# HenryHZY/VL-PET

Measured on AMD Instinct MI355X. Metric: multitask samples/sec (BART-base, r=96), higher is better.
Workload: dtype bf16

## Files before the change

### include/vlpet_hip.h

```cpp
#ifndef VLPET_HIP_H
#define VLPET_HIP_H
#include <stddef.h>
#include <stdint.h>

#ifdef __cplusplus
extern "C" {
#endif

#define VLPET_F32 0
#define VLPET_BF16 1

#define VLPET_E_SHAPE (-1)
#define VLPET_E_RANK (-2)
#define VLPET_E_ALIGN (-3)
#define VLPET_E_WORKSPACE (-4)
#define VLPET_E_NULL (-5)
#define VLPET_E_DTYPE (-6)
#define VLPET_E_ALIAS (-7)

#define VLPET_GATE_NONE 0
#define VLPET_GATE_MUL 1
#define VLPET_GATE_ADD 2

typedef void* vlpet_stream_t;
// ... 302 lines not shown
                      int64_t bs_v, const void* k_new, const void* v_new, int64_t ld_new, int pos, const uint8_t* key_mask,
                      int64_t ld_mask, const float* bias, int64_t ld_bias, void* o, int64_t ld_o, int B, int H, int D, int Lk,
                      float scale, int io_dtype, vlpet_stream_t stream);
int vlpet_greedy_pick(const void* logits, int64_t ld, int V, int64_t* ids, int64_t ld_ids, int pos, int* unfinished, int* counter,
                      int B, int eos_token_id, int pad_token_id, int min_length, int no_repeat_ngram_size, int io_dtype,
                      vlpet_stream_t stream);

int vlpet_attn_decode_beam(const void* q, int64_t ld_q, void* k_cache, void* v_cache, int64_t ld_k, int64_t bs_k, int64_t ld_v,
                           int64_t bs_v, const void* k_new, const void* v_new, int64_t ld_new, int pos, const uint8_t* key_mask,
                           int64_t ld_mask, const float* bias, int64_t ld_bias, void* o, int64_t ld_o, int B, int H, int D,
                           int Lk, float scale, int group, const int* key_rows, int64_t ld_key_rows, int io_dtype,
                           vlpet_stream_t stream);
int vlpet_beam_rows(const void* logits, int64_t ld, int V, const int64_t* ids, int64_t ld_ids, int pos, int rows, int num_beams,
                    int slices, int eos_token_id, int min_length, int no_repeat_ngram_size, int force_eos, float* part_stats,
                    float* part_val, int* part_tok, int io_dtype, vlpet_stream_t stream);
int vlpet_beam_advance(const float* part_stats, const float* part_val, const int* part_tok, int slices, int V, int B, int num_beams,
                       float* beam_scores, const int64_t* ids_in, int64_t* ids_out, int64_t ld_ids, const int* key_rows_in,
                       int* key_rows_out, int64_t ld_key_rows, int64_t* next_tokens, float* hyp_score, int* hyp_meta,
                       int64_t* hyp_tokens, int64_t ld_hyp, float* item_worst, int* item_state, int* counter, int pos,
                       int eos_token_id, int pad_token_id, float length_penalty, int early_stopping, vlpet_stream_t stream);

int vlpet_attn_decode_at(const void* q, int64_t ld_q, void* k_cache, void* v_cache, int64_t ld_k, int64_t bs_k, int64_t ld_v,
                         int64_t bs_v, const void* k_new, const void* v_new, int64_t ld_new, const int* pos_dev, int pos_limit,
                         const uint8_t* key_mask, int64_t ld_mask, const float* bias, int64_t ld_bias, int64_t pos_stride_bias,
                         void* o, int64_t ld_o, int B, int H, int D, int Lk, float scale, const int* key_rows,
                         int64_t ld_key_rows, int64_t parity_stride_key_rows, int io_dtype, vlpet_stream_t stream);
int vlpet_greedy_pick_at(const void* logits, int64_t ld, int V, int64_t* ids, int64_t ld_ids, const int* pos_dev, int pos_limit,
                         int* unfinished, int* counters, int64_t* next_tokens, int B, int eos_token_id, int pad_token_id,
                         int min_length, int no_repeat_ngram_size, int io_dtype, vlpet_stream_t stream);
int vlpet_beam_rows_at(const void* logits, int64_t ld, int V, const int64_t* ids, int64_t ld_ids, int64_t parity_stride_ids,
                       const int* pos_dev, int pos_limit, int rows, int num_beams, int slices, int eos_token_id, int min_length,
                       int no_repeat_ngram_size, int force_eos_pos, float* part_stats, float* part_val, int* part_tok,
                       int io_dtype, vlpet_stream_t stream);
int vlpet_beam_advance_at(const float* part_stats, const float* part_val, const int* part_tok, int slices, int V, int B,
                          int num_beams, float* beam_scores, int64_t* ids, int64_t ld_ids, int64_t parity_stride_ids,
                          int* key_rows, int64_t ld_key_rows, int64_t parity_stride_key_rows, int64_t* next_tokens,
                          float* hyp_score, int* hyp_meta, int64_t* hyp_tokens, int64_t ld_hyp, float* item_worst, int* item_state,
                          int* counters, const int* pos_dev, int pos_limit, int eos_token_id, int pad_token_id,
                          float length_penalty, int early_stopping, vlpet_stream_t stream);

int vlpet_adapter_tail_rows(void);
int vlpet_adapter_tail_applies(int64_t M, int d, int r, int io_dtype);
int vlpet_adapter_tail_fwd(const void* h, const void* res, const void* down_w, const void* down_b, const void* up_w,
                           const void* up_b, const float* gamma, const float* beta, void* out, int64_t M, int d, int r,
                           float scale, float eps, int norm_mode, int param_dtype, int io_dtype, vlpet_stream_t stream);

size_t vlpet_phm_workspace_bytes(int d, int r, int n);
int vlpet_phm_expand_pair_fwd(const void* rule_d, const void* W_d, const void* rule_u, const void* W_u, void* wt_d, void* wt_u,
                              int d, int r, int n, int param_dtype, vlpet_stream_t stream);
int vlpet_phm_expand_pair_bwd(const float* dwt_d, const float* dwt_u, const void* rule_d, const void* W_d, const void* rule_u,
                              const void* W_u, float* drule_d, float* dW_d, float* drule_u, float* dW_u, void* workspace,
                              size_t workspace_bytes, int d, int r, int n, int param_dtype, vlpet_stream_t stream);

#ifdef __cplusplus
}
#endif
#endif
```

### vl-pet_amd/_lib.py

```python
from __future__ import annotations

import ctypes
import os
from ctypes import c_char_p, c_float, c_int, c_int64, c_size_t, c_uint64, c_void_p

_HERE = os.path.dirname(os.path.abspath(__file__))
LIB_PATH = os.environ.get("VLPET_LIB") or os.path.join(_HERE, "lib", "libvlpet_hip.so")

VLPET_F32 = 0
VLPET_BF16 = 1
GATE_NONE, GATE_MUL, GATE_ADD = 0, 1, 2

_lib = None

SIGNATURES = {
    "vlpet_version": (c_int, []),
    "vlpet_error_string": (c_char_p, [c_int]),
    "vlpet_rank_tiles": (c_int, [c_int]),
    "vlpet_packed_bytes": (c_size_t, [c_int, c_int, c_int]),
    "vlpet_pack_pair": (c_int, [c_void_p, c_void_p, c_int, c_void_p, c_void_p, c_int, c_int, c_int, c_int, c_int,
                                c_void_p, c_void_p]),
    "vlpet_pack_pairs": (c_int, [c_int, c_void_p, c_void_p, c_int, c_void_p, c_void_p, c_int, c_int, c_int, c_int, c_int,
                                 c_void_p, c_void_p]),
    "vlpet_adapter_gate_fwd": (c_int, [c_void_p, c_void_p, c_void_p, c_void_p, c_void_p, c_int64, c_int, c_int,
# ... 99 lines not shown
    "vlpet_attn_bwd": (c_int, [c_void_p] * 10 + [c_int] * 5 + [c_float, c_float, c_uint64, c_void_p]),
    "vlpet_attn_fwd_ld": (c_int, [c_void_p] * 7 + [c_int] * 7 + [c_float, c_float, c_uint64, c_void_p]),
    "vlpet_attn_bwd_ld": (c_int, [c_void_p] * 10 + [c_int] * 7 + [c_float, c_float, c_uint64, c_void_p]),
    "vlpet_attn_fwd_bias": (c_int, [c_void_p] * 8 + [c_int] * 7 + [c_float, c_float, c_uint64, c_void_p]),
    "vlpet_attn_bwd_bias": (c_int, [c_void_p] * 12 + [c_int] * 7 + [c_float, c_float, c_uint64, c_void_p]),
    "vlpet_concat_dropout_fwd": (c_int, [c_void_p] * 3 + [c_int64, c_int, c_int, c_int, c_float, c_uint64, c_int, c_void_p]),
    "vlpet_concat_dropout_bwd": (c_int, [c_void_p] * 3 + [c_int64, c_int, c_int, c_int, c_float, c_uint64, c_int, c_void_p]),
    "vlpet_prefix_concat_chunks": (c_int, [c_int64]),
    "vlpet_prefix_concat_ws_bytes": (c_size_t, [c_int64, c_int, c_int]),
    "vlpet_prefix_concat_dropout_fwd": (c_int, [c_void_p] * 4 + [c_int64, c_int, c_int, c_int, c_int, c_float, c_uint64, c_int, c_void_p]),
    "vlpet_prefix_concat_dropout_bwd": (c_int, [c_void_p] * 5 + [c_int64, c_int, c_int, c_int, c_int, c_float, c_uint64, c_int, c_void_p]),
    "vlpet_attn_fwd_kv": (c_int, [c_void_p] * 8 + [c_int] * 8 + [c_float, c_float, c_uint64, c_void_p]),
    "vlpet_attn_bwd_kv": (c_int, [c_void_p] * 12 + [c_int] * 8 + [c_float, c_float, c_uint64, c_void_p]),
    "vlpet_attn_long_fwd": (c_int, [c_void_p] * 7 + [c_int] * 8 + [c_float, c_void_p]),
    "vlpet_attn_long_fwd_train": (c_int, [c_void_p] * 8 + [c_int] * 8 + [c_float, c_float, c_uint64, c_void_p]),
    "vlpet_attn_long_bwd": (c_int, [c_void_p] * 12 + [c_int] * 8 + [c_float, c_float, c_uint64, c_void_p, c_void_p]),
    "vlpet_ce_loss_fwd": (c_int, [c_void_p] * 4 + [c_int64, c_int, c_int, c_int, c_void_p]),
    "vlpet_ce_loss_fwd_checked": (c_int, [c_void_p] * 5 + [c_int64, c_int, c_int, c_int, c_void_p]),
    "vlpet_ce_loss_bwd": (c_int, [c_void_p] * 5 + [c_int64, c_int, c_int, c_int, c_void_p]),
    "vlpet_act_dropout_fwd": (c_int, [c_void_p] * 3 + [c_int64, c_int, c_float, c_uint64, c_int, c_void_p]),
    "vlpet_act_dropout_bwd": (c_int, [c_void_p] * 3 + [c_int64, c_int, c_float, c_uint64, c_int, c_void_p]),
    "vlpet_attn_decode": (c_int, [c_void_p, c_int64, c_void_p, c_void_p, c_int64, c_int64, c_int64, c_int64, c_void_p, c_void_p,
                                  c_int64, c_int, c_void_p, c_int64, c_void_p, c_int64, c_void_p, c_int64, c_int, c_int, c_int,
                                  c_int, c_float, c_int, c_void_p]),
    "vlpet_greedy_pick": (c_int, [c_void_p, c_int64, c_int, c_void_p, c_int64, c_int, c_void_p, c_void_p, c_int, c_int, c_int,
                                  c_int, c_int, c_int, c_void_p]),
    "vlpet_attn_decode_beam": (c_int, [c_void_p, c_int64, c_void_p, c_void_p, c_int64, c_int64, c_int64, c_int64, c_void_p,
                                       c_void_p, c_int64, c_int, c_void_p, c_int64, c_void_p, c_int64, c_void_p, c_int64, c_int,
                                       c_int, c_int, c_int, c_float, c_int, c_void_p, c_int64, c_int, c_void_p]),
    "vlpet_beam_rows": (c_int, [c_void_p, c_int64, c_int, c_void_p, c_int64, c_int, c_int, c_int, c_int, c_int, c_int, c_int, c_int,
                                c_void_p, c_void_p, c_void_p, c_int, c_void_p]),
    "vlpet_beam_advance": (c_int, [c_void_p, c_void_p, c_void_p, c_int, c_int, c_int, c_int, c_void_p, c_void_p, c_void_p, c_int64,
                                   c_void_p, c_void_p, c_int64, c_void_p, c_void_p, c_void_p, c_void_p, c_int64, c_void_p,
                                   c_void_p, c_void_p, c_int, c_int, c_int, c_float, c_int, c_void_p]),
    "vlpet_attn_decode_at": (c_int, [c_void_p, c_int64, c_void_p, c_void_p, c_int64, c_int64, c_int64, c_int64, c_void_p, c_void_p,
                                     c_int64, c_void_p, c_int, c_void_p, c_int64, c_void_p, c_int64, c_int64, c_void_p, c_int64,
                                     c_int, c_int, c_int, c_int, c_float, c_void_p, c_int64, c_int64, c_int, c_void_p]),
    "vlpet_greedy_pick_at": (c_int, [c_void_p, c_int64, c_int, c_void_p, c_int64, c_void_p, c_int, c_void_p, c_void_p, c_void_p,
                                     c_int, c_int, c_int, c_int, c_int, c_int, c_void_p]),
    "vlpet_beam_rows_at": (c_int, [c_void_p, c_int64, c_int, c_void_p, c_int64, c_int64, c_void_p, c_int, c_int, c_int, c_int, c_int,
                                   c_int, c_int, c_int, c_void_p, c_void_p, c_void_p, c_int, c_void_p]),
    "vlpet_beam_advance_at": (c_int, [c_void_p, c_void_p, c_void_p, c_int, c_int, c_int, c_int, c_void_p, c_void_p, c_int64, c_int64,
                                      c_void_p, c_int64, c_int64, c_void_p, c_void_p, c_void_p, c_void_p, c_int64, c_void_p,
                                      c_void_p, c_void_p, c_void_p, c_int, c_int, c_int, c_float, c_int, c_void_p]),
    "vlpet_adapter_tail_rows": (c_int, []),
    "vlpet_adapter_tail_applies": (c_int, [c_int64, c_int, c_int, c_int]),
    "vlpet_adapter_tail_fwd": (c_int, [c_void_p] * 9 + [c_int64, c_int, c_int, c_float, c_float, c_int, c_int, c_int, c_void_p]),
    "vlpet_lora_delta_bwd": (c_int, [c_void_p, c_void_p, c_void_p, c_void_p, c_float, c_uint64, c_void_p, c_void_p,
                                     c_void_p, c_int, c_void_p, c_size_t, c_int64, c_int, c_int, c_float, c_int,
                                     c_void_p]),
    "vlpet_phm_workspace_bytes": (c_size_t, [c_int, c_int, c_int]),
    "vlpet_phm_expand_pair_fwd": (c_int, [c_void_p] * 6 + [c_int, c_int, c_int, c_int, c_void_p]),
    "vlpet_phm_expand_pair_bwd": (c_int, [c_void_p] * 11 + [c_size_t, c_int, c_int, c_int, c_int, c_void_p]),
}


def load():
    global _lib
    if _lib is not None:
        return _lib
    if not os.path.exists(LIB_PATH):
        raise RuntimeError(
            f"vl-pet_amd: HIP library not found at {LIB_PATH}; run `python -c 'import __graft_entry__ as g; "
            f"g.build()'` (there is no CPU fallback for the PET hot path)")
    import torch
    if torch.cuda.is_available():
        torch.cuda.init()
    lib = ctypes.CDLL(LIB_PATH)
    for name, (res, args) in SIGNATURES.items():
        fn = getattr(lib, name)
        fn.restype = res
        fn.argtypes = args
    _lib = lib
    return lib


def check(code: int, what: str):
    if code != 0:
        msg = load().vlpet_error_string(code)
        raise RuntimeError(f"vl-pet_amd: {what} failed: {msg.decode() if msg else code} (code {code})")
```

### vl-pet_amd/csrc/api.hip

```cpp
#include <atomic>
#include "../../include/vlpet_hip.h"
#include "common.h"
#include "kernels.h"
#include <cmath>
#include <stdlib.h>
#include <stdio.h>
#include <vector>

#define VLPET_VERSION 680
#define VLPET_VERSION_R3 300
#define VLPET_VERSION_R2 221

static inline bool aligned16(const void* p) { return (reinterpret_cast<uintptr_t>(p) & 15) == 0; }
static inline size_t align256(size_t v) { return (v + 255) / 256 * 256; }
static inline int herr(hipError_t e) { return e == hipSuccess ? 0 : (int)e; }

extern "C" int vlpet_version(void) { return VLPET_VERSION; }
extern "C" int vlpet_debug_build(void) { return VLPET_IS_DEBUG_BUILD; }

__global__ __launch_bounds__(64) void hold_cus_kernel(unsigned* release, unsigned long long ticks) {
    extern __shared__ __attribute__((aligned(16))) uint8_t hold_smem[];
    typedef __attribute__((address_space(1))) unsigned gu32;
    if (threadIdx.x == 0) {
        hold_smem[0] = 1;
        const unsigned long long t0 = wall_clock64();
        while (__hip_atomic_load((gu32*)release, __ATOMIC_RELAXED, __HIP_MEMORY_SCOPE_AGENT) == 0u && wall_clock64() - t0 < ticks)
            __builtin_amdgcn_s_sleep(32);
    }
}
extern "C" int vlpet_test_hold_cus(int workgroups, int lds_bytes, void* release_flag, int max_ms, vlpet_stream_t stream) {
    if (!release_flag) return VLPET_E_NULL;
    if (workgroups <= 0 || workgroups > 1024 || lds_bytes < 0 || lds_bytes > 160 * 1024 || max_ms <= 0) return VLPET_E_SHAPE;
    if (max_ms > 10000) max_ms = 10000;
    hipError_t e = hipFuncSetAttribute(reinterpret_cast<const void*>(hold_cus_kernel), hipFuncAttributeMaxDynamicSharedMemorySize, lds_bytes);
    if (e != hipSuccess) return herr(e);
    hipLaunchKernelGGL(hold_cus_kernel, dim3((unsigned)workgroups), dim3(64), (size_t)lds_bytes, (hipStream_t)stream,
                       reinterpret_cast<unsigned*>(release_flag), (unsigned long long)max_ms * 100000ull);
    return herr(hipGetLastError());
}

extern "C" const char* vlpet_error_string(int code) {
    switch (code) {
        case 0: return "success";
        case VLPET_E_SHAPE: return "bad shape (need M > 0, d % 64 == 0, r > 0)";
        case VLPET_E_RANK: return "unsupported bottleneck rank (max 192) or tile count";
        case VLPET_E_ALIGN: return "pointer not 16-byte aligned";
        case VLPET_E_WORKSPACE: return "workspace too small";
        case VLPET_E_NULL: return "required pointer is NULL";
        case VLPET_E_DTYPE: return "unsupported dtype";
        case VLPET_E_ALIAS: return "output overlaps an input";
        default: return code > 0 ? hipGetErrorString((hipError_t)code) : "unknown error";
    }
}

extern "C" int vlpet_rank_tiles(int r) {
    if (r <= 0) return VLPET_E_SHAPE;
    if (r <= 32) return 1;
    if (r <= 96) return 3;
    if (r <= 192) return 6;
    return VLPET_E_RANK;
}

// ... 1589 lines not shown
extern "C" size_t vlpet_phm_workspace_bytes(int d, int r, int n) { return phm_geometry(d, r, n) == 0 ? phm_ws_bytes(d, r, n) : 0; }

struct ByteRange { const void* p; size_t bytes; };
static bool phm_outputs_alias(const ByteRange* in, int n_in, const ByteRange* out, int n_out) {
    for (int o = 0; o < n_out; ++o) {
        const uintptr_t x = reinterpret_cast<uintptr_t>(out[o].p);
        for (int i = 0; i < n_in + n_out; ++i) {
            if (i >= n_in && i - n_in <= o) continue;
            const ByteRange& q = i < n_in ? in[i] : out[i - n_in];
            const uintptr_t y = reinterpret_cast<uintptr_t>(q.p);
            if (x < y + q.bytes && y < x + out[o].bytes) return true;
        }
    }
    return false;
}

extern "C" int vlpet_phm_expand_pair_fwd(const void* rule_d, const void* W_d, const void* rule_u, const void* W_u, void* wt_d, void* wt_u,
                                         int d, int r, int n, int param_dtype, vlpet_stream_t stream) {
    if (!rule_d || !W_d || !rule_u || !W_u || !wt_d || !wt_u) return VLPET_E_NULL;
    if (!dtype_ok(param_dtype)) return VLPET_E_DTYPE;
    if (int rc = phm_geometry(d, r, n)) return rc;
    if (!aligned16(rule_d) || !aligned16(W_d) || !aligned16(rule_u) || !aligned16(W_u) || !aligned16(wt_d) || !aligned16(wt_u))
        return VLPET_E_ALIGN;
    const size_t es = param_dtype == VLPET_F32 ? 4 : 2, nr = (size_t)n * n * n * es, nw = (size_t)d * r / n * es, nh = (size_t)d * r * es;
    const ByteRange in[4] = {{rule_d, nr}, {W_d, nw}, {rule_u, nr}, {W_u, nw}}, out[2] = {{wt_d, nh}, {wt_u, nh}};
    if (phm_outputs_alias(in, 4, out, 2)) return VLPET_E_ALIAS;
    PhmArgs a{};
    a.l[0].rule = rule_d; a.l[0].W = W_d; a.l[0].wt = wt_d; a.l[0].in = d; a.l[0].out = r;
    a.l[1].rule = rule_u; a.l[1].W = W_u; a.l[1].wt = wt_u; a.l[1].in = r; a.l[1].out = d;
    a.n = n;
    return herr(launch_phm_expand_fwd(a, param_dtype == VLPET_F32, (hipStream_t)stream));
}

extern "C" int vlpet_phm_expand_pair_bwd(const float* dwt_d, const float* dwt_u, const void* rule_d, const void* W_d, const void* rule_u,
                                         const void* W_u, float* drule_d, float* dW_d, float* drule_u, float* dW_u, void* workspace,
                                         size_t workspace_bytes, int d, int r, int n, int param_dtype, vlpet_stream_t stream) {
    if (!dwt_d || !dwt_u || !rule_d || !W_d || !rule_u || !W_u || !drule_d || !dW_d || !drule_u || !dW_u || !workspace) return VLPET_E_NULL;
    if (!dtype_ok(param_dtype)) return VLPET_E_DTYPE;
    if (int rc = phm_geometry(d, r, n)) return rc;
    if (!aligned16(dwt_d) || !aligned16(dwt_u) || !aligned16(rule_d) || !aligned16(W_d) || !aligned16(rule_u) || !aligned16(W_u) ||
        !aligned16(drule_d) || !aligned16(dW_d) || !aligned16(drule_u) || !aligned16(dW_u) || !aligned16(workspace)) return VLPET_E_ALIGN;
    const size_t need = phm_ws_bytes(d, r, n);
    if (workspace_bytes < need) return VLPET_E_WORKSPACE;
    const size_t es = param_dtype == VLPET_F32 ? 4 : 2, n3 = (size_t)n * n * n, nw = (size_t)d * r / n, nh = (size_t)d * r;
    const ByteRange in[6] = {{dwt_d, nh * 4}, {dwt_u, nh * 4}, {rule_d, n3 * es}, {W_d, nw * es}, {rule_u, n3 * es}, {W_u, nw * es}};
    const ByteRange out[5] = {{drule_d, n3 * 4}, {dW_d, nw * 4}, {drule_u, n3 * 4}, {dW_u, nw * 4}, {workspace, need}};
    if (phm_outputs_alias(in, 6, out, 5)) return VLPET_E_ALIAS;
    PhmArgs a{};
    a.l[0].rule = rule_d; a.l[0].W = W_d; a.l[0].dwt = dwt_d; a.l[0].drule = drule_d; a.l[0].dW = dW_d; a.l[0].in = d; a.l[0].out = r;
    a.l[1].rule = rule_u; a.l[1].W = W_u; a.l[1].dwt = dwt_u; a.l[1].drule = drule_u; a.l[1].dW = dW_u; a.l[1].in = r; a.l[1].out = d;
    a.n = n; a.ws = reinterpret_cast<float*>(workspace);
    return herr(launch_phm_expand_bwd(a, param_dtype == VLPET_F32, (hipStream_t)stream));
}
```

### vl-pet_amd/csrc/kernels.h

```cpp
#pragma once
#include <cstdlib>
#include <hip/hip_runtime.h>
#include <stdint.h>
#include "rng.h"
#include "tuning.h"

#define VLPET_MAX_HEADS 16

struct PackArgs {
    const void* wd[VLPET_MAX_HEADS];
    const void* bd[VLPET_MAX_HEADS];
    const void* wu;
    const void* bu;
    int n_heads, rows_per_head;
    int r, d, RT;
    int src_bf16;
    int n_packs;
    uint8_t* out;
};
hipError_t launch_pack_pair(const PackArgs& a, int NS, hipStream_t stream);
#define VLPET_PACK_BATCH 8
struct PackBatch { PackArgs p[VLPET_PACK_BATCH]; int n; };
hipError_t launch_pack_pairs(const PackBatch& b, int NS, hipStream_t stream);

// ... 375 lines not shown
    uint8_t* keep_out;
    int B, H, Lq, Lk, causal;
    int ld_q, ld_kv;
    int ld_v;
    float scale;
    uint32_t thr;
    float inv_keep;
    uint64_t seed;
    const uint64_t* seed_ctr;
    int dbg;
};
size_t attn_lds_bytes(int Lq, int Lk, int bwd);
hipError_t launch_attn(const AttnArgs& a, bool bwd, hipStream_t stream);
hipError_t launch_attn_bwd_fewq(const AttnArgs& a, hipStream_t stream);
hipError_t launch_attn_long_fwd(const AttnArgs& a, hipStream_t stream);
hipError_t launch_attn_long_bwd(const AttnArgs& a, float* delta, hipStream_t stream);

struct AdapterTailArgs {
    const void* h;
    const void* res;
    const void* wd;
    const void* bd;
    const void* wu;
    const void* bu;
    const float* gamma;
    const float* beta;
    void* out;
    int64_t M;
    int d, r;
    float scale, eps;
    int norm;
};
int adapter_tail_rows(void);
bool adapter_tail_geometry_ok(int d, int r);
hipError_t launch_adapter_tail(const AdapterTailArgs& a, int io_fp32, int param_fp32, hipStream_t stream);

struct PhmLayer {
    const void* rule;
    const void* W;
    void* wt;
    const float* dwt;
    float* drule;
    float* dW;
    int in, out;
};
struct PhmArgs {
    PhmLayer l[2];
    int n;
    float* ws;
};
int64_t phm_layer_tiles(int in, int out, int n);
hipError_t launch_phm_expand_fwd(const PhmArgs& a, int param_fp32, hipStream_t stream);
hipError_t launch_phm_expand_bwd(const PhmArgs& a, int param_fp32, hipStream_t stream);
```

### vl-pet_amd/functional.py

```python
from __future__ import annotations

import ctypes
from typing import Optional, Sequence

import torch
import torch.nn.functional as F

from . import _lib

GATE_NONE, GATE_MUL, GATE_ADD = _lib.GATE_NONE, _lib.GATE_MUL, _lib.GATE_ADD


class KernelTimer:

    def __init__(self, names=None):
        self.records = []
        self.names = None if names is None else frozenset(names)

    def wants(self, name):
        return self.names is None or name in self.names

    def bracket(self, name, rows, fn):
        e0 = torch.cuda.Event(enable_timing=True)
        e1 = torch.cuda.Event(enable_timing=True)
# ... 378 lines not shown
                dx = t if dx is None else dx.add_(t)
        return (None if dx is None else dx.view(ctx.xshape)), None, None, None, None


def cross_key_blocks(x: torch.Tensor, w_all: torch.Tensor, b_all: torch.Tensor, n: int):
    from .attention import KeyGradSlot
    slot = KeyGradSlot(n, w_all.shape[0] // n) if (x.requires_grad and torch.is_grad_enabled()) else None
    return _CrossKeyProjFn.apply(x, w_all, b_all, n, slot), slot


class ResidualLink:

    __slots__ = ("armed", "_grad", "_shared")

    def __init__(self):
        self.armed = False
        self._grad = None
        self._shared = False

    def arm(self) -> "ResidualLink":
        self.armed = True
        return self

    @staticmethod
    def if_armed(link: Optional["ResidualLink"]) -> Optional["ResidualLink"]:
        return link if (link is not None and link.armed) else None

    @property
    def holds(self) -> bool:
        return self._grad is not None

    def park(self, grad: torch.Tensor, shared: bool = False):
        if self._grad is not None:
            raise RuntimeError("vl-pet_amd: a gradient is already parked in this ResidualLink (it would be lost)")
        self._grad, self._shared = grad, bool(shared)

    def take(self, shape, dtype, writable: bool = False) -> Optional[torch.Tensor]:
        g, shared = self._grad, self._shared
        self._grad, self._shared = None, False
        if g is None:
            return None
        parked = g
        if g.shape != shape:
            g = g.reshape(shape)
        if g.dtype != dtype:
            g = g.to(dtype)
        if not g.is_contiguous():
            g = g.contiguous()
        if writable and shared and g.data_ptr() == parked.data_ptr():
            g = g.clone()
        return g


class _LinearAccFn(torch.autograd.Function):

    @staticmethod
    def forward(ctx, x, link, *wb):
        n = len(wb) // 2
        ws, bs = wb[:n], wb[n:]
        ctx.link = link.arm() if (link is not None and ctx.needs_input_grad[0]) else None
        ctx.save_for_backward(*ws)
        ctx.xshape = x.shape
        outs = tuple(F.linear(x, w, b) for w, b in zip(ws, bs))
        return outs if n > 1 else outs[0]

    @staticmethod
    def backward(ctx, *dys):
        ws = ctx.saved_tensors
        link, ctx.link = ctx.link, None
        acc = link.take(ctx.xshape, ws[0].dtype, writable=True) if link is not None else None
        if acc is not None:
            acc = acc.view(-1, ctx.xshape[-1])
        for dy, w in zip(dys, ws):
            if dy is None:
                continue
            dy2 = dy.reshape(-1, dy.shape[-1])
            if dy2.dtype != w.dtype:
                dy2 = dy2.to(w.dtype)
            if acc is None:
                acc = dy2 @ w
            else:
                acc.addmm_(dy2, w)
        dx = acc.view(ctx.xshape) if acc is not None else None
        return (dx, None) + (None,) * (2 * len(ws))


def io_view(p: torch.Tensor, dtype: torch.dtype) -> torch.Tensor:
    if p.dtype == dtype:
        return p
    sh = getattr(p, "_vlpet_io", None)
    if sh is not None and sh[0].io_epoch == WEIGHTS_EPOCH and sh[1].dtype == dtype:
        return sh[1]
    return p.to(dtype)


class _LinearTrainBiasFn(torch.autograd.Function):

    @staticmethod
    def forward(ctx, x, w, b, link=None):
        ctx.link = link.arm() if (link is not None and ctx.needs_input_grad[0]) else None
        ctx.save_for_backward(w, b)
        return F.linear(x, w, io_view(b, x.dtype))

    @staticmethod
    def backward(ctx, dy):
        lib = _lib.load()
        w, b = ctx.saved_tensors
        n = dy.shape[-1]
        dy2 = _flat(dy, n)
        if dy2.dtype != w.dtype:
            dy2 = dy2.to(w.dtype)
        dx = None
        link, ctx.link = ctx.link, None
        if ctx.needs_input_grad[0]:
            xshape = (*dy.shape[:-1], w.shape[1])
            base = link.take(xshape, w.dtype, writable=True) if link is not None else None
            if base is not None:
                dx = base.view(-1, w.shape[1]).addmm_(dy2, w).view(xshape)
            else:
                dx = (dy2 @ w).view(xshape)
        db = None
        if ctx.needs_input_grad[2]:
            M = dy2.shape[0]
            slot = grad_slot(b, (n,))
            nb = lib.vlpet_sublayer_tail_partials(M)
            ws = torch.empty(nb * n, dtype=torch.float32, device=dy2.device)
            if DEFER_REDUCES and slot.sunk:
                rc = lib.vlpet_colsum_partial(dy2.data_ptr(), M, n, ws.data_ptr(), _io_dtype(dy2), _stream())
                _lib.check(rc, "vlpet_colsum_partial")
                tf = slot.t.reshape(-1)
                reduce_partials(ws, nb, n // 2, tf[:n // 2], tf[n // 2:], True)
            else:
                rc = lib.vlpet_colsum(dy2.data_ptr(), M, n, ws.data_ptr(), slot.ptr, _io_dtype(dy2), _stream())
                _lib.check(rc, "vlpet_colsum")
            db = slot.finish()
        return dx, None, db, None

# ... 334 lines not shown
```

### vl-pet_amd/host/bart.py

```python
from __future__ import annotations

import copy
import math
from types import SimpleNamespace

import torch
import torch.nn as nn
import torch.nn.functional as F

from .. import attention as A
from .. import decode as D
from .. import functional as VF
from .. import adapter_tail as AT
from ..adapters import AdapterController
from ..encoder_pet import apply_pet, build_pet, has_pet
from ..lora import LoRALinearController, LoraConfig
from ..visual import Downsample, LowRankVisualEmbedding, VisualEmbedding
from ..prompt import PromptController
from .common import (COMPACTER_DEFAULTS, PROMPT_DEFAULTS, check_sequential_adapter_flags, derived_weights, eval_no_grad, fused_adapter_tail,
                     install_shared_phm_rule, is_key_mask, make_adapter_config, make_prompt_config, sequential_adapters, shift_right, unpack_vis_inputs,
                     value_parallel_adapter)

TASKS = ["vqa", "gqa", "nlvr", "caption"]

# ... 97 lines not shown
    if (link is not None and FUSE_BIAS_GRAD and isinstance(mod, nn.Linear) and not mod.weight.requires_grad and mod.bias is not None
            and mod.bias.requires_grad):
        w = mod.weight if mod.weight.dtype == x.dtype else mod.weight.to(x.dtype)
        if VF.linear_train_bias_ok(x, w, mod.bias):
            return VF.linear_train_bias(x, w, mod.bias, link)
    return _linear(mod, x)


def sublayer_tail(residual, h, norm, p, training, link=None):
    from ..tail import sublayer_tail as _hip_tail
    return _hip_tail(residual, h, norm, p, training, link=link)


def _tail_linked(residual, h, norm, p, training, link):
    link = VF.ResidualLink.if_armed(link)
    if link is None:
        return sublayer_tail(residual, h, norm, p, training)
    return sublayer_tail(residual, h, norm, p, training, link=link)


def ffn_activation(x, act, p, training):
    if EAGER_FFN_ACT:
        return F.dropout(F.gelu(x) if act == "gelu" else F.relu(x), p=p, training=training)
    from ..act import act_dropout
    return act_dropout(x, act, p, training)


EAGER_FFN_ACT = False


def lm_loss(h, weight, labels, bias=None):
    if EAGER_LM_LOSS:
        logits = F.linear(h, weight.to(h.dtype))
        if bias is not None:
            logits = logits + bias.to(h.dtype)
        loss = F.cross_entropy(logits.float().view(-1, logits.shape[-1]), labels.view(-1), ignore_index=-100, reduction="none")
        return loss.view(labels.shape), logits
    from ..lmloss import lm_head_loss
    return lm_head_loss(h, weight, labels, bias)


EAGER_LM_LOSS = False


def _linear(mod: nn.Linear, x):
    w, b = mod.weight, mod.bias
    if w.dtype != x.dtype:
        w = w.to(x.dtype)
    if FUSE_BIAS_GRAD and b is not None and b.requires_grad:
        if VF.linear_train_bias_ok(x, w, b):
            return VF.linear_train_bias(x, w, b)
    if b is not None and b.dtype != x.dtype:
        b = b.to(x.dtype)
    return F.linear(x, w, b)


def _sdpa_ctx():
    import contextlib
    which = SDPA_BACKEND
    if not which:
        return contextlib.nullcontext()
    from torch.nn.attention import SDPBackend, sdpa_kernel
    return sdpa_kernel({"flash": SDPBackend.FLASH_ATTENTION, "efficient": SDPBackend.EFFICIENT_ATTENTION,
                        "math": SDPBackend.MATH}[which])


def attention_core(q, k, v, num_heads, attn_mask, causal, p, training, k_slot=None):
    B, Lq, E = q.shape
    kind = _route(Lq, k.shape[1], p, training, q, k, v) if attn_mask is None or is_key_mask(attn_mask) else None
    if A.fits(kind, q, k, v, num_heads):
        km = None if attn_mask is None else attn_mask[:, 0, 0, :]
        return A.attend(kind, q, k, v, num_heads, km, causal and attn_mask is None, p, training, k_slot=k_slot)
    sh = lambda t: t.reshape(B, -1, num_heads, E // num_heads).transpose(1, 2)
    with _sdpa_ctx():
        out = F.scaled_dot_product_attention(sh(q), sh(k), sh(v), attn_mask=attn_mask, is_causal=causal and attn_mask is None,
                                             dropout_p=p if training else 0.0)
    return out.transpose(1, 2).reshape(B, Lq, E)


FUSE_BIAS_GRAD = True
EAGER_ATTENTION = False
LONG_ATTENTION = False
LONG_ATTENTION_TRAIN = False


def _route(Lq, Lk, p, training, *tensors, grad=False):
    return A.route(Lq, Lk, p, training, A.needs_grad(*tensors, grad=grad), eager=EAGER_ATTENTION, long_on=LONG_ATTENTION,
                   long_train_on=LONG_ATTENTION_TRAIN)


def _long_applies(Lq, Lk, p, training, *tensors) -> bool:
    return _route(Lq, Lk, p, training, *tensors) == "long"


def _long_train_applies(Lq, Lk, p, training, *tensors, grad=False) -> bool:
    return _route(Lq, Lk, p, training, *tensors, grad=grad) == "long_train"
FUSE_QKV = True
FUSE_CROSS_KEYS = True
SDPA_BACKEND = None


class BartAttention(nn.Module):

    def __init__(self, config, embed_dim, num_heads, dropout, is_cross=False, value_adapter=False):
        super().__init__()
        self.embed_dim, self.num_heads, self.dropout = embed_dim, num_heads, dropout
# ... 402 lines not shown
```

Before: 29510.

## Add custom HIP row-GEMM kernel for frozen BART linears with shape routing

Adds a hand-written bf16 MFMA GEMM kernel with a multi-slot LDS ring pipeline, swizzled layout and a fused bias or accumulate epilogue. It serves forward and input-gradient products for frozen BART linear layers. A route table limits its use to particular (M,N,K) ranges, and every other shape falls back to hipBLASLt/torch. The intent is to beat the vendor GEMM at the small and medium row counts seen in PET training, at the cost of more code, per-call host routing checks, and bf16 rounding of the accumulate path.

```diff
diff --git a/include/vlpet_hip.h b/include/vlpet_hip.h
--- a/include/vlpet_hip.h
+++ b/include/vlpet_hip.h
@@ -378,6 +378,12 @@
                               const void* W_u, float* drule_d, float* dW_d, float* drule_u, float* dW_u, void* workspace,
                               size_t workspace_bytes, int d, int r, int n, int param_dtype, vlpet_stream_t stream);
 
+int vlpet_linear_rows_fwd(const void* x, const void* w, const void* bias, void* out, int64_t M, int N, int K, int dtype,
+                          vlpet_stream_t stream);
+int vlpet_linear_rows_dgrad(const void* dy, const void* w, void* dx, int64_t M, int N, int K, int accumulate, int dtype,
+                            vlpet_stream_t stream);
+int vlpet_linear_rows_route(int64_t M, int N, int K, int direction, int accumulate, int dtype);
+
 #ifdef __cplusplus
 }
 #endif
diff --git a/vl-pet_amd/_lib.py b/vl-pet_amd/_lib.py
--- a/vl-pet_amd/_lib.py
+++ b/vl-pet_amd/_lib.py
@@ -175,6 +175,9 @@
     "vlpet_phm_workspace_bytes": (c_size_t, [c_int, c_int, c_int]),
     "vlpet_phm_expand_pair_fwd": (c_int, [c_void_p] * 6 + [c_int, c_int, c_int, c_int, c_void_p]),
     "vlpet_phm_expand_pair_bwd": (c_int, [c_void_p] * 11 + [c_size_t, c_int, c_int, c_int, c_int, c_void_p]),
+    "vlpet_linear_rows_fwd": (c_int, [c_void_p] * 4 + [c_int64, c_int, c_int, c_int, c_void_p]),
+    "vlpet_linear_rows_dgrad": (c_int, [c_void_p] * 3 + [c_int64, c_int, c_int, c_int, c_int, c_void_p]),
+    "vlpet_linear_rows_route": (c_int, [c_int64, c_int, c_int, c_int, c_int, c_int]),
 }
 
 
diff --git a/vl-pet_amd/csrc/api.hip b/vl-pet_amd/csrc/api.hip
--- a/vl-pet_amd/csrc/api.hip
+++ b/vl-pet_amd/csrc/api.hip
@@ -7,7 +7,7 @@
 #include <stdio.h>
 #include <vector>
 
-#define VLPET_VERSION 680
+#define VLPET_VERSION 690
 #define VLPET_VERSION_R3 300
 #define VLPET_VERSION_R2 221
 
@@ -1703,3 +1703,45 @@
     a.n = n; a.ws = reinterpret_cast<float*>(workspace);
     return herr(launch_phm_expand_bwd(a, param_dtype == VLPET_F32, (hipStream_t)stream));
 }
+
+static int linrows_common(const void* a, const void* w, const void* out, const void* bias, int64_t M, int N, int K, int dtype) {
+    if (!a || !w || !out || M <= 0 || M > ((int64_t)1 << 24)) return VLPET_E_SHAPE;
+    if (!linrows_shape_ok(N, K)) return VLPET_E_RANK;
+    if (!aligned16(a) || !aligned16(w) || !aligned16(out) || (bias && !aligned16(bias))) return VLPET_E_ALIGN;
+    if (dtype != VLPET_BF16) return VLPET_E_DTYPE;
+    return 0;
+}
+extern "C" int vlpet_linear_rows_fwd(const void* x, const void* w, const void* bias, void* out, int64_t M, int N, int K, int dtype,
+                                     vlpet_stream_t stream) {
+    const int rc = linrows_common(x, w, out, bias, M, N, K, dtype);
+    if (rc) return rc;
+    LinRowsArgs a{};
+    a.a = x; a.w = w; a.bias = bias; a.out = out; a.M = M; a.Kc = K; a.NO = N; a.ldw = K; a.accumulate = 0;
+    return herr(launch_linear_rows(a, false, (hipStream_t)stream));
+}
+extern "C" int vlpet_linear_rows_dgrad(const void* dy, const void* w, void* dx, int64_t M, int N, int K, int accumulate, int dtype,
+                                       vlpet_stream_t stream) {
+    const int rc = linrows_common(dy, w, dx, nullptr, M, N, K, dtype);
+    if (rc) return rc;
+    LinRowsArgs a{};
+    a.a = dy; a.w = w; a.bias = nullptr; a.out = dx; a.M = M; a.Kc = N; a.NO = K; a.ldw = K; a.accumulate = accumulate ? 1 : 0;
+    return herr(launch_linear_rows(a, true, (hipStream_t)stream));
+}
+struct LinRowsRoute { int dgrad, accumulate, N, K; int64_t lo, hi; };
+static const LinRowsRoute LINROWS_ROUTES[] = {
+    {0, 0, 768, 768, 1040, 1932},
+    {0, 0, 2304, 768, 42, 315},
+    {1, 0, 768, 768, 42, 2500},
+    {1, 0, 2304, 768, 1040, 2500},
+    {1, 0, 768, 3072, 42, 315},
+    {1, 1, 768, 768, 42, 315},
+    {1, 1, 768, 768, 525, 2500},
+    {1, 1, 768, 3072, 42, 315},
+};
+extern "C" int vlpet_linear_rows_route(int64_t M, int N, int K, int direction, int accumulate, int dtype) {
+    if (dtype != VLPET_BF16 || M <= 0 || !linrows_shape_ok(N, K) || direction < 0 || direction > 1) return 0;
+    if (direction == 0 && accumulate) return 0;
+    for (const LinRowsRoute& r : LINROWS_ROUTES)
+        if (r.dgrad == direction && r.accumulate == (accumulate ? 1 : 0) && r.N == N && r.K == K && M >= r.lo && M <= r.hi) return 1;
+    return 0;
+}
diff --git a/vl-pet_amd/csrc/kernels.h b/vl-pet_amd/csrc/kernels.h
--- a/vl-pet_amd/csrc/kernels.h
+++ b/vl-pet_amd/csrc/kernels.h
@@ -451,3 +451,17 @@
 int64_t phm_layer_tiles(int in, int out, int n);
 hipError_t launch_phm_expand_fwd(const PhmArgs& a, int param_fp32, hipStream_t stream);
 hipError_t launch_phm_expand_bwd(const PhmArgs& a, int param_fp32, hipStream_t stream);
+
+struct LinRowsArgs {
+    const void* a;
+    const void* w;
+    const void* bias;
+    void* out;
+    int64_t M;
+    int Kc, NO, ldw;
+    int accumulate;
+};
+constexpr int64_t LINR_M_SMALL = 1280, LINR_M_MID = 6144;
+bool linrows_shape_ok(int N, int K);
+int linrows_form(int64_t M);
+hipError_t launch_linear_rows(const LinRowsArgs& a, bool dgrad, hipStream_t stream);
diff --git a/vl-pet_amd/csrc/linear_rows.hip b/vl-pet_amd/csrc/linear_rows.hip
--- /dev/null
+++ b/vl-pet_amd/csrc/linear_rows.hip
@@ -0,0 +1,251 @@
+#include "cols_common.h"
+#include "kernels.h"
+
+constexpr int LINR_BN = 128;
+
+template <int BM> struct LinRowsGeo {
+    static constexpr int NSLOT = BM == 32 ? 6 : BM == 64 ? 4 : 3;
+    static constexpr int XT_B = BM * 128, WT_B = LINR_BN * 128, STG_B = XT_B + WT_B;
+    static constexpr int PX = BM / 8, NP = PX + 16, NPW = NP / 4;
+    static constexpr int RING_B = NSLOT * STG_B;
+    static constexpr int OUT_B = BM * LINR_BN * 2;
+    static constexpr int LDS_B = RING_B > OUT_B ? RING_B : OUT_B;
+    static_assert(PX % 4 == 0 && LDS_B <= 160 * 1024, "");
+};
+
+__device__ __forceinline__ int linr_sw(int row) { return (row >> 1) & 7; }
+template <int NI, int MAXA>
+__device__ __forceinline__ void linr_wait(int ahead) {
+    static_assert(MAXA >= 1 && MAXA <= 5, "");
+    if (ahead >= MAXA) wgs_wait_n<MAXA * NI>();
+    else if (ahead <= 0) wgs_wait_n<0>();
+    else if (ahead == 1) wgs_wait_n<NI>();
+    else if (ahead == 2) wgs_wait_n<(MAXA > 2 ? 2 : 1) * NI>();
+    else if (ahead == 3) wgs_wait_n<(MAXA > 3 ? 3 : 1) * NI>();
+    else wgs_wait_n<(MAXA > 4 ? 4 : 1) * NI>();
+}
+
+template <int BM, int WM, bool DGRAD>
+__global__ __launch_bounds__(256) void linrows_kernel(LinRowsArgs a) {
+    using GEO = LinRowsGeo<BM>;
+    constexpr int WN = 4 / WM, RT = BM / (32 * WM), FT = LINR_BN / (32 * WN);
+    constexpr int XT_B = GEO::XT_B, STG_B = GEO::STG_B, PX = GEO::PX, NPW = GEO::NPW, NSLOT = GEO::NSLOT;
+    static_assert(RT >= 1 && RT <= 2 && FT >= 1 && FT <= 2, "");
+    extern __shared__ __attribute__((aligned(16))) uint8_t smem[];
+
+    const int tid = threadIdx.x, lane = tid & 63, wave = __builtin_amdgcn_readfirstlane(tid >> 6);
+    const int wm = wave / WN, wn = wave % WN;
+    const int n = lane & 31, kh = lane >> 5;
+    const uint32_t lds0 = (uint32_t)(uintptr_t)(__attribute__((address_space(3))) uint8_t*)smem;
+
+    const int NCB = a.NO / LINR_BN;
+    const int rb = (int)blockIdx.x / NCB, cb = (int)blockIdx.x % NCB;
+    const int64_t row0 = (int64_t)rb * BM;
+    const int c0 = cb * LINR_BN;
+    const int last = (int)(a.M - row0 < BM ? a.M - row0 : BM) - 1;
+    const int lda2 = a.Kc * 2, ldw2 = a.ldw * 2, ldo2 = a.NO * 2;
+    const int T = a.Kc / 64;
+    const uint8_t* Ap = reinterpret_cast<const uint8_t*>(a.a) + row0 * lda2;
+    const uint8_t* Wp = reinterpret_cast<const uint8_t*>(a.w) + (DGRAD ? (int64_t)c0 * 2 : (int64_t)c0 * ldw2);
+    const int64_t wstep = DGRAD ? (int64_t)64 * ldw2 : 128;
+
+    const int lr = lane >> 3, ls = lane & 7;
+    uint32_t poff[NPW];
+    sfor<NPW>([&](auto IC) {
+        constexpr int i = decltype(IC)::value;
+        const int p = 4 * i + wave;
+        if constexpr (i < PX / 4) {
+            const int row = 8 * p + lr;
+            const int rc = row > last ? last : row;
+            poff[i] = (uint32_t)rc * (uint32_t)lda2 + (uint32_t)((ls ^ linr_sw(row)) * 16);
+        } else {
+            const int pw = p - PX;
+            if constexpr (DGRAD) {
+                const int h = pw >> 3, r = 8 * (pw & 7) + lr;
+                poff[i] = (uint32_t)r * (uint32_t)ldw2 + (uint32_t)(h * 128 + ((ls ^ fsw(r)) * 16));
+            } else {
+                const int row = 8 * pw + lr;
+                poff[i] = (uint32_t)row * (uint32_t)ldw2 + (uint32_t)((ls ^ linr_sw(row)) * 16);
+            }
+        }
+    });
+    auto issue = [&](int s) {
+        uint8_t* st = smem + (size_t)(s % NSLOT) * STG_B;
+        const uint8_t* xs = sbase(Ap + (int64_t)s * 128);
+        const uint8_t* ws = sbase(Wp + (int64_t)s * wstep);
+        sfor<NPW>([&](auto IC) {
+            constexpr int i = decltype(IC)::value;
+            if constexpr (i < PX / 4) glds16(xs + poff[i], st + (4 * i + wave) * 1024);
+            else glds16(ws + poff[i], st + XT_B + (4 * i + wave - PX) * 1024);
+        });
+    };
+
+    uint32_t foff[4];
+#pragma unroll
+    for (int u = 0; u < 4; ++u) foff[u] = (uint32_t)(((2 * u + kh) ^ linr_sw(n)) * 16);
+    const uint32_t xbase = (uint32_t)((wm * RT * 32 + n) * 128);
+    const uint32_t wbase = (uint32_t)(XT_B + (wn * FT * 32 + n) * 128);
+    uint32_t a_wtr[FT][2];
+    {
+        const int g4 = lane >> 4, sl = lane & 15;
+        const int trow = 8 * (g4 >> 1) + (sl >> 2);
+        const int tslot = 2 * (g4 & 1) + ((sl & 3) >> 1), thalf = 8 * (sl & 1);
+#pragma unroll
+        for (int ft = 0; ft < FT; ++ft) {
+            const int coloff = wn * FT * 32 + ft * 32, h = coloff >> 6, nt = (coloff >> 5) & 1;
+#pragma unroll
+            for (int hi = 0; hi < 2; ++hi) {
+                const int r = trow + 4 * hi;
+                a_wtr[ft][hi] = (uint32_t)(XT_B + h * 8192 + r * 128 + (((4 * nt + tslot) ^ fsw(r)) * 16) + thalf);
+            }
+        }
+    }
+
+    f32x16 acc[FT][RT];
+#pragma unroll
+    for (int ft = 0; ft < FT; ++ft)
+#pragma unroll
+        for (int rt = 0; rt < RT; ++rt) acc[ft][rt] = zero16();
+
+#pragma unroll
+    for (int s = 0; s < NSLOT - 1; ++s) issue(s);
+
+    constexpr int RPU = (DGRAD ? 2 * FT : FT) + RT;
+#pragma unroll 1
+    for (int t = 0; t < T; ++t) {
+        int ahead = T - 1 - t;
+        if (ahead > NSLOT - 2) ahead = NSLOT - 2;
+        linr_wait<NPW, NSLOT - 2>(ahead);
+        __builtin_amdgcn_s_barrier();
+        const uint32_t sb = lds0 + (uint32_t)((t % NSLOT) * STG_B);
+        u32x4 xf[4][RT], wf[4][FT];
+        TrOp wt[4][FT];
+        sfor<4>([&](auto UC) {
+            constexpr int u = decltype(UC)::value;
+            sfor<FT>([&](auto F) {
+                if constexpr (DGRAD) tr_read2<u * 16 * 128>(wt[u][F.value], sb + a_wtr[F.value][0], sb + a_wtr[F.value][1]);
+                else lds_read16<F.value * 32 * 128>(wf[u][F.value], sb + wbase + foff[u]);
+            });
+            sfor<RT>([&](auto R) { lds_read16<R.value * 32 * 128>(xf[u][R.value], sb + xbase + foff[u]); });
+        });
+        if (t + NSLOT - 1 < T) issue(t + NSLOT - 1);
+        sfor<2>([&](auto HC) {
+            constexpr int hf = decltype(HC)::value;
+            if constexpr (hf == 0) asm volatile("s_waitcnt lgkmcnt(%0)" :: "n"(2 * RPU) : "memory");
+            else asm volatile("s_waitcnt lgkmcnt(0)" ::: "memory");
+            sfor<2>([&](auto UH) {
+                constexpr int u = 2 * hf + decltype(UH)::value;
+#pragma unroll
+                for (int ft = 0; ft < FT; ++ft) { if constexpr (DGRAD) tr_tie(wt[u][ft]); else lgkm_tie(wf[u][ft]); }
+#pragma unroll
+                for (int rt = 0; rt < RT; ++rt) lgkm_tie(xf[u][rt]);
+#pragma unroll
+                for (int ft = 0; ft < FT; ++ft) {
+                    bf16x8 af;
+                    if constexpr (DGRAD) af = tr_val(wt[u][ft]); else af = as_bf(wf[u][ft]);
+#pragma unroll
+                    for (int rt = 0; rt < RT; ++rt) acc[ft][rt] = mfma32(af, as_bf(xf[u][rt]), acc[ft][rt]);
+                }
+            });
+            __builtin_amdgcn_sched_barrier(0);
+        });
+    }
+    asm volatile("s_waitcnt vmcnt(0) lgkmcnt(0)" ::: "memory");
+    __syncthreads();
+
+    uint8_t* Op = reinterpret_cast<uint8_t*>(a.out) + row0 * ldo2 + (int64_t)c0 * 2;
+    constexpr int NLINE = BM * 16 / 256;
+    const bool accum = DGRAD && a.accumulate != 0;
+    const __bf16* bias = DGRAD ? nullptr : reinterpret_cast<const __bf16*>(a.bias);
+    if (accum) {
+        u32x4 cv[NLINE];
+#pragma unroll
+        for (int i = 0; i < NLINE; ++i) {
+            const int idx = tid + 256 * i, row = idx >> 4, slot = idx & 15;
+            const int rc = row > last ? last : row;
+            cv[i] = *reinterpret_cast<const u32x4*>(Op + (int64_t)rc * ldo2 + slot * 16);
+        }
+#pragma unroll
+        for (int i = 0; i < NLINE; ++i) {
+            const int idx = tid + 256 * i, row = idx >> 4, slot = idx & 15;
+            *reinterpret_cast<u32x4*>(smem + row * 256 + ((slot ^ (row & 7)) * 16)) = cv[i];
+        }
+        __syncthreads();
+    }
+    auto round_tile = [&](auto HB, auto HA) {
+        constexpr bool HAS_BIAS = decltype(HB)::value, HAS_ACC = decltype(HA)::value;
+        u32x2 b2[FT][4];
+        if constexpr (HAS_BIAS) {
+#pragma unroll
+            for (int ft = 0; ft < FT; ++ft)
+#pragma unroll
+                for (int q = 0; q < 4; ++q) b2[ft][q] = *reinterpret_cast<const u32x2*>(bias + c0 + (wn * FT + ft) * 32 + 8 * q + 4 * kh);
+        }
+#pragma unroll
+        for (int rt = 0; rt < RT; ++rt) {
+            const int row = (wm * RT + rt) * 32 + n;
+#pragma unroll
+            for (int ft = 0; ft < FT; ++ft) {
+#pragma unroll
+                for (int q = 0; q < 4; ++q) {
+                    const int f = (wn * FT + ft) * 32 + 8 * q + 4 * kh;
+                    uint8_t* ad = smem + row * 256 + (((f >> 3) ^ (row & 7)) * 16) + 8 * kh;
+                    float o[4];
+#pragma unroll
+                    for (int j = 0; j < 4; ++j) o[j] = acc[ft][rt][4 * q + j];
+                    if constexpr (HAS_BIAS) {
+                        o[0] += bf_lo(b2[ft][q][0]); o[1] += bf_hi(b2[ft][q][0]); o[2] += bf_lo(b2[ft][q][1]); o[3] += bf_hi(b2[ft][q][1]);
+                    }
+                    if constexpr (HAS_ACC) {
+                        const u32x2 c2 = *reinterpret_cast<const u32x2*>(ad);
+                        o[0] += bf_lo(c2[0]); o[1] += bf_hi(c2[0]); o[2] += bf_lo(c2[1]); o[3] += bf_hi(c2[1]);
+                    }
+                    typedef __attribute__((ext_vector_type(4))) __bf16 bf16x4;
+                    const bf16x4 t4 = {(__bf16)o[0], (__bf16)o[1], (__bf16)o[2], (__bf16)o[3]};
+                    *reinterpret_cast<u32x2*>(ad) = __builtin_bit_cast(u32x2, t4);
+                }
+            }
+        }
+    };
+    if (bias) round_tile(std::true_type{}, std::false_type{});
+    else if (accum) round_tile(std::false_type{}, std::true_type{});
+    else round_tile(std::false_type{}, std::false_type{});
+    __syncthreads();
+    {
+        u32x4 ov[NLINE];
+#pragma unroll
+        for (int i = 0; i < NLINE; ++i) {
+            const int idx = tid + 256 * i, row = idx >> 4, slot = idx & 15;
+            ov[i] = *reinterpret_cast<const u32x4*>(smem + row * 256 + ((slot ^ (row & 7)) * 16));
+        }
+#pragma unroll
+        for (int i = 0; i < NLINE; ++i) {
+            const int idx = tid + 256 * i, row = idx >> 4, slot = idx & 15;
+            if (row <= last) *reinterpret_cast<u32x4*>(Op + (int64_t)row * ldo2 + slot * 16) = ov[i];
+        }
+    }
+}
+
+bool linrows_shape_ok(int N, int K) {
+    return (N == 768 && K == 768) || (N == 2304 && K == 768) || (N == 3072 && K == 768) || (N == 768 && K == 3072);
+}
+int linrows_form(int64_t M) { return M <= LINR_M_SMALL ? 32 : M <= LINR_M_MID ? 64 : 128; }
+
+template <int BM, int WM, bool DGRAD>
+static hipError_t linrows_go(const LinRowsArgs& a, hipStream_t stream) {
+    using GEO = LinRowsGeo<BM>;
+    auto kern = linrows_kernel<BM, WM, DGRAD>;
+    hipError_t e = hipFuncSetAttribute(reinterpret_cast<const void*>(kern), hipFuncAttributeMaxDynamicSharedMemorySize, GEO::LDS_B);
+    if (e != hipSuccess) return e;
+    const unsigned grid = (unsigned)((a.M + BM - 1) / BM) * (unsigned)(a.NO / LINR_BN);
+    hipLaunchKernelGGL(kern, dim3(grid), dim3(256), GEO::LDS_B, stream, a);
+    return hipGetLastError();
+}
+
+hipError_t launch_linear_rows(const LinRowsArgs& a, bool dgrad, hipStream_t stream) {
+    switch (linrows_form(a.M)) {
+        case 32: return dgrad ? linrows_go<32, 1, true>(a, stream) : linrows_go<32, 1, false>(a, stream);
+        case 64: return dgrad ? linrows_go<64, 2, true>(a, stream) : linrows_go<64, 2, false>(a, stream);
+        default: return dgrad ? linrows_go<128, 2, true>(a, stream) : linrows_go<128, 2, false>(a, stream);
+    }
+}
diff --git a/vl-pet_amd/functional.py b/vl-pet_amd/functional.py
--- a/vl-pet_amd/functional.py
+++ b/vl-pet_amd/functional.py
@@ -454,6 +454,47 @@
         return g
 
 
+HIP_ROW_GEMM = True
+_ROW_ROUTES: dict = {}
+
+
+def _row_route(M: int, N: int, K: int, direction: int, accumulate: int) -> bool:
+    key = (M, N, K, direction, accumulate)
+    r = _ROW_ROUTES.get(key)
+    if r is None:
+        r = _ROW_ROUTES[key] = bool(_lib.load().vlpet_linear_rows_route(M, N, K, direction, accumulate, _lib.VLPET_BF16))
+    return r
+
+
+def _row_operand_ok(*ts) -> bool:
+    return all(t is None or (t.is_cuda and t.dtype == torch.bfloat16 and t.is_contiguous() and t.data_ptr() % 16 == 0) for t in ts)
+
+
+def _rows_fwd(x: torch.Tensor, w: torch.Tensor, b: Optional[torch.Tensor]) -> torch.Tensor:
+    N, K = w.shape
+    if HIP_ROW_GEMM and x.dim() >= 2 and x.shape[-1] == K and x.numel() > 0 and _row_operand_ok(x, w, b):
+        M = x.numel() // K
+        if _row_route(M, N, K, 0, 0):
+            out = torch.empty((*x.shape[:-1], N), dtype=x.dtype, device=x.device)
+            rc = _lib.load().vlpet_linear_rows_fwd(x.data_ptr(), w.data_ptr(), b.data_ptr() if b is not None else None, out.data_ptr(),
+                                                   M, N, K, _lib.VLPET_BF16, _stream())
+            _lib.check(rc, "vlpet_linear_rows_fwd")
+            return out
+    return F.linear(x, w, b)
+
+
+def _rows_dgrad(dy2: torch.Tensor, w: torch.Tensor, acc: Optional[torch.Tensor]) -> torch.Tensor:
+    N, K = w.shape
+    M = dy2.shape[0]
+    if HIP_ROW_GEMM and M > 0 and _row_operand_ok(dy2, w, acc) and _row_route(M, N, K, 1, 0 if acc is None else 1):
+        dx = acc if acc is not None else torch.empty((M, K), dtype=dy2.dtype, device=dy2.device)
+        rc = _lib.load().vlpet_linear_rows_dgrad(dy2.data_ptr(), w.data_ptr(), dx.data_ptr(), M, N, K, 0 if acc is None else 1,
+                                                 _lib.VLPET_BF16, _stream())
+        _lib.check(rc, "vlpet_linear_rows_dgrad")
+        return dx
+    return dy2 @ w if acc is None else acc.addmm_(dy2, w)
+
+
 class _LinearAccFn(torch.autograd.Function):
 
     @staticmethod
@@ -463,7 +504,7 @@
         ctx.link = link.arm() if (link is not None and ctx.needs_input_grad[0]) else None
         ctx.save_for_backward(*ws)
         ctx.xshape = x.shape
-        outs = tuple(F.linear(x, w, b) for w, b in zip(ws, bs))
+        outs = tuple(_rows_fwd(x, w, b) for w, b in zip(ws, bs))
         return outs if n > 1 else outs[0]
 
     @staticmethod
@@ -479,12 +520,20 @@
             dy2 = dy.reshape(-1, dy.shape[-1])
             if dy2.dtype != w.dtype:
                 dy2 = dy2.to(w.dtype)
-            if acc is None:
-                acc = dy2 @ w
-            else:
-                acc.addmm_(dy2, w)
+            acc = _rows_dgrad(dy2, w, acc)
         dx = acc.view(ctx.xshape) if acc is not None else None
         return (dx, None) + (None,) * (2 * len(ws))
+
+
+def frozen_linear(x: torch.Tensor, w: torch.Tensor, b: Optional[torch.Tensor], link: Optional["ResidualLink"] = None) -> torch.Tensor:
+    if link is None:
+        N, K = w.shape
+        M = x.numel() // K if K else 0
+        grad = x.requires_grad and torch.is_grad_enabled()
+        if not (HIP_ROW_GEMM and M > 0 and _row_operand_ok(x, w, b)
+                and (_row_route(M, N, K, 0, 0) or (grad and _row_route(M, N, K, 1, 0)))):
+            return F.linear(x, w, b)
+    return _LinearAccFn.apply(x, link, w, b)
 
 
 def io_view(p: torch.Tensor, dtype: torch.dtype) -> torch.Tensor:
diff --git a/vl-pet_amd/host/bart.py b/vl-pet_amd/host/bart.py
--- a/vl-pet_amd/host/bart.py
+++ b/vl-pet_amd/host/bart.py
@@ -173,6 +173,8 @@
             return VF.linear_train_bias(x, w, b)
     if b is not None and b.dtype != x.dtype:
         b = b.to(x.dtype)
+    if not w.requires_grad and (b is None or not b.requires_grad):
+        return VF.frozen_linear(x, w, b)
     return F.linear(x, w, b)
 
 
```

Result: no change. 29500 (-0.0%).
